# Sthiber/COSC_4397_Pathtracing_Raytracing_Project

Measured on AMD Instinct MI355X. Metric: Msamples/s, cornell.txt 1920x1080 depth 8 (+PSNR vs 5000spp ref), higher is better.
Workload: dtype f32

## Files before the change

### cosc_4397_pathtracing_raytracing_project_amd/csrc/pt_kernels.hip

```cpp
#include "pt_kernels.h"

#include <float.h>

#include <type_traits>

#include "pt_lds.h"
#include "pt_sched.h"
#include "pt_portable_math.h"

#ifndef PT_ARITH
#define PT_ARITH 0
#endif
#if PT_ARITH == 0
#define PT_NS arith_exact
#define PT_API_FN api_exact
#elif PT_ARITH == 1
#define PT_NS arith_fma
#define PT_API_FN api_fma
#elif PT_ARITH == 2
#define PT_NS arith_fast
#define PT_API_FN api_fast
#else
#error "PT_ARITH must be 0, 1 or 2"
#endif
// ... 8 lines not shown
constexpr bool kFloatTrig = PT_ARITH == 1;

#ifdef PT_WALK_STATS
__device__ unsigned long long g_walk_stats[16];
#define PT_STAT(i, v)                                                             \
  do {                                                                            \
    const unsigned long long pt_stat_v = (unsigned long long)(v);  \
    if (lane_id() == 0) atomicAdd(&g_walk_stats[i], pt_stat_v);                   \
  } while (0)
PT_DEV int wave_max_stat(int v) {
  for (int o = 32; o; o >>= 1) v = max(v, __shfl_xor(v, o));
  return v;
}
#else
#define PT_STAT(i, v)
#endif

constexpr int kStealMin = 16;
constexpr int kPrimaryWaves = 5;

typedef float v4f __attribute__((ext_vector_type(4)));
struct f3 {
  float x, y, z;
};
PT_DEV unsigned long long ballot(bool p) { return __builtin_amdgcn_ballot_w64(p); }
PT_DEV uint32_t push_bit(uint32_t m, bool bit) {
  uint32_t r;
  unsigned long long carry_out;
  asm("v_addc_co_u32_e64 %0, %1, %2, %2, %3" : "=v"(r), "=s"(carry_out) : "v"(m), "s"(ballot(bit)));
  return r;
}
PT_DEV int rank_in(unsigned long long m) { return __builtin_amdgcn_mbcnt_hi((uint32_t)(m >> 32), __builtin_amdgcn_mbcnt_lo((uint32_t)m, 0)); }
PT_DEV f3 mk(float x, float y, float z) { return f3{x, y, z}; }

#include "pt_ieee.inc"
PT_DEV void divmod(int a, int n, float inv_n, int& q, int& r) {
  int k = (int)((float)a * inv_n);
  int rem = a - k * n;
  if (rem < 0) {
    rem += n;
    --k;
  } else if (rem >= n) {
    rem -= n;
    ++k;
  }
  q = k;
  r = rem;
}

struct RayInv {
  float ix, iy, iz;
  bool sx, sy, sz;
  float nx, ny, nz;
};

}

#pragma clang fp contract(off)
namespace ex {
namespace {
constexpr bool kFastArith = false, kFusedRef = false;
#include "pt_arith.inc"
}
}
#if PT_ARITH != 0
#pragma clang fp contract(fast)
#endif
namespace md {
namespace {
constexpr bool kFastArith = kFast, kFusedRef = PT_ARITH == 1;
#include "pt_arith.inc"
}
}
namespace {
using namespace md;
constexpr bool kD0 = PT_ARITH != 0;
template <bool EX>
struct Ar {
  static PT_DEV RayInv ray_inv(f3 d, f3 o) { if constexpr (EX) return ex::ray_inv(d, o); else return md::ray_inv(d, o); }
  static PT_DEV bool slab(f3 o, const RayInv& ri, float a, float b, float c, float d, float e, float f) {
    if constexpr (EX) return ex::slab(o, ri, a, b, c, d, e, f); else return md::slab(o, ri, a, b, c, d, e, f);
  }
  static PT_DEV bool slab_rel(const RayInv& ri, float a, float b, float c, float d, float e, float f) {
    if constexpr (EX) return ex::slab_rel(ri, a, b, c, d, e, f); else return md::slab_rel(ri, a, b, c, d, e, f);
  }
  static PT_DEV bool slab_t(f3 o, const RayInv& ri, float a, float b, float c, float d, float e, float f, float& tn) {
    if constexpr (EX) return ex::slab_t(o, ri, a, b, c, d, e, f, tn); else return md::slab_t(o, ri, a, b, c, d, e, f, tn);
  }
  template <int TYPE, bool QO, bool DEFER = false>
  static PT_DEV float geom_test(const ptd::Geom* __restrict__ G, f3 ro, f3 rd, f3& point, f3& normal, f3 qo_pre, int rt_type = -1) {
    if constexpr (EX) return ex::geom_test<TYPE, QO, DEFER>(G, ro, rd, point, normal, qo_pre, rt_type);
    else return md::geom_test<TYPE, QO, DEFER>(G, ro, rd, point, normal, qo_pre, rt_type);
  }
  static PT_DEV f3 finish_normal(const ptd::Geom* __restrict__ G, f3 stored) {
    if constexpr (EX) return ex::finish_normal(G, stored); else return md::finish_normal(G, stored);
  }
  static PT_DEV f3 camera_dir(const ptd::Camera& cam, float inv_w, int p, bool aa, float jx, float jy) {
    if constexpr (EX) return ex::camera_dir(cam, inv_w, p, aa, jx, jy); else return md::camera_dir(cam, inv_w, p, aa, jx, jy);
  }
  static PT_DEV f3 xf_point(const float* m, f3 v) { if constexpr (EX) return ex::mulMV<1>(m, v); else return md::mulMV<1>(m, v); }
};

PT_DEV int lane_id() { return (int)(threadIdx.x & 63); }
PT_DEV float bperm(int src_lane, float v) {
  return __int_as_float(__builtin_amdgcn_ds_bpermute(src_lane << 2, __float_as_int(v)));
}

PT_DEV uint32_t utilhash(uint32_t a) {
  a = (a + 0x7ed55d16u) + (a << 12);
  a = (a ^ 0xc761c23cu) ^ (a >> 19);
  a = (a + 0x165667b1u) + (a << 5);
  a = (a + 0xd3a2646cu) ^ (a << 9);
  a = (a + 0xfd7046c5u) + (a << 3);
  a = (a ^ 0xb55a4f09u) ^ (a >> 16);
  return a;
}
struct MinStd {
  uint32_t x;
  PT_DEV explicit MinStd(uint32_t s) {
    uint32_t r = (s & 0x7fffffffu) + (s >> 31);
    if (r >= 0x7fffffffu) r -= 0x7fffffffu;
    x = r == 0u ? 1u : r;
  }
  PT_DEV uint32_t next() {
    uint64_t p = (uint64_t)x * 48271u;
    uint32_t r = (uint32_t)(p & 0x7fffffffu) + (uint32_t)(p >> 31);
    if (r >= 0x7fffffffu) r -= 0x7fffffffu;
    x = r;
    return r;
  }
  PT_DEV float u01() { return (float)(next() - 1u) * 4.656612873077392578125e-10f; }
};
PT_DEV uint32_t iter_hash(int iter, int depth) { return utilhash((1u << 31) | ((uint32_t)depth << 22) | (uint32_t)iter); }
PT_DEV void iter_hash_fill(uint32_t* tab, const SceneTables& sc, const BatchInfo& b, int depth) {
  if (iter_hash_entries(sc) > 0)
    for (int i = threadIdx.x; i < b.K; i += blockDim.x) tab[i] = iter_hash(b.iter_first + i, depth);
}
PT_DEV uint32_t iter_hash_of(const uint32_t* tab, const SceneTables& sc, const BatchInfo& b, int depth, int k) {
  return iter_hash_entries(sc) > 0 ? tab[k] : iter_hash(b.iter_first + k, depth);
}

PT_DEV void aa_jitter(int iter, int pixel, float& jx, float& jy) {
  MinStd rng(utilhash((1u << 31) | (1u << 30) | (uint32_t)iter) ^ utilhash((uint32_t)pixel));
  jx = rng.u01() - 0.5f;
  jy = rng.u01() - 0.5f;
}

PT_DEV void stage16(void* lds, const void* g, int bytes) {
  const float4* src = reinterpret_cast<const float4*>(g);
  float4* dst = reinterpret_cast<float4*>(lds);
  for (int i = threadIdx.x; i < bytes / 16; i += blockDim.x) dst[i] = src[i];
}

PT_DEV int global_pixel(const BatchInfo& b, int p) {
  if (b.stripe == 0) return b.pixel_begin + p;
  if (b.list) return b.pixel_begin + b.list[p];
  int i, r;
  divmod(p, b.stripe, b.inv_stripe, i, r);
  return b.pixel_begin + p + i * b.gap;
}

struct PathTag {
  int slot;
  uint32_t phash;
  int k;
};
struct PathRec {
  f3 o, d, c;
  PathTag tag;
};
struct alignas(8) Word2 {
  float x, y;
};
PT_DEV void plane2_load(const ptd::PathBuf& b, int64_t at, float& cz, PathTag& tag) {
  const Word2 w2 = reinterpret_cast<const Word2*>(b.r + 2 * b.stride)[at];
  cz = w2.x;
  tag.slot = __float_as_int(w2.y), tag.phash = 0u, tag.k = 0;
}
PT_DEV void plane2_store(const ptd::PathBuf& b, int64_t at, float cz, const PathTag& tag) {
  reinterpret_cast<Word2*>(b.r + 2 * b.stride)[at] = Word2{cz, __int_as_float(tag.slot)};
}
PT_DEV void path_load_ray(const ptd::PathBuf& b, int64_t at, f3& o, f3& d) {
  const ptd::Word4 w0 = b.r[at], w1 = b.r[b.stride + at];
  o = mk(w0.x, w0.y, w0.z);
  d = mk(w0.w, w1.x, w1.y);
}
PT_DEV void path_load_tail(const ptd::PathBuf& b, int64_t at, f3& d, f3& c, PathTag& tag) {
  const ptd::Word4 w1 = b.r[b.stride + at];
  float cz;
  plane2_load(b, at, cz, tag);
  d = mk(reinterpret_cast<const float*>(b.r + at)[3], w1.x, w1.y);
  c = mk(w1.z, w1.w, cz);
}
PT_DEV PathRec path_load(const ptd::PathBuf& b, int64_t at) {
  const ptd::Word4 w0 = b.r[at], w1 = b.r[b.stride + at];
  PathRec v;
  float cz;
  plane2_load(b, at, cz, v.tag);
  v.o = mk(w0.x, w0.y, w0.z);
  v.d = mk(w0.w, w1.x, w1.y);
  v.c = mk(w1.z, w1.w, cz);
  return v;
}
PT_DEV void path_store(const ptd::PathBuf& b, int64_t at, f3 o, f3 d, f3 c, const PathTag& tag) {
  b.r[at] = ptd::Word4{o.x, o.y, o.z, d.x};
  b.r[b.stride + at] = ptd::Word4{d.y, d.z, c.x, c.y};
  plane2_store(b, at, c.z, tag);
}
PT_DEV int make_slot(const BatchInfo& b, int k, int pl) { return (k << b.slot_shift) | pl; }
PT_DEV void sample_of(const PathTag& tag, const BatchInfo& b, int& k, int& pl) {
  k = (int)((uint32_t)tag.slot >> b.slot_shift);
  pl = tag.slot & ((1 << b.slot_shift) - 1);
}
PT_DEV uint32_t path_seed(int k, int pl, const uint32_t* ihash, const SceneTables& sc, const BatchInfo& b, int depth) {
  return iter_hash_of(ihash, sc, b, depth, k) ^ utilhash((uint32_t)global_pixel(b, pl));
}

struct Retire {
  ptd::Word4* rec;
  unsigned long long* sub;
  unsigned long long* cnt;
  int seg_cap, wq0;
};
PT_DEV Retire retire_of(const ptd::RetireBuf& rb, int q) {
  Retire rt;
  rt.rec = rb.rec + (int64_t)q * rb.kmax * rb.seg_cap;
  rt.sub = rb.sub + (int64_t)q * rb.kmax * rb.wq0;
  rt.cnt = rb.cnt + (int64_t)q * rb.kmax;
  rt.seg_cap = rb.seg_cap, rt.wq0 = rb.wq0;
  return rt;
}
PT_DEV void retire_store(const Retire& rt, bool dead, int k, int pos, int pl, f3 c) {
  if (dead) rt.rec[(int64_t)k * rt.seg_cap + pos] = ptd::Word4{c.x, c.y, c.z, __int_as_float(pl)};
}
PT_DEV void retire_append(const Retire& rt, bool dead, int k, int pl, f3 c) {
  if (dead) retire_store(rt, true, k, (int)(atomicAdd(&rt.cnt[k], 1ull << 32) >> 32), pl, c);
}

__global__ __launch_bounds__(kBlock) void k_generate(ptd::Camera cam, BatchInfo b, ptd::Queues qs, ptd::PathBuf out,
                                                     int32_t* __restrict__ cnt0) {
  const int wave = blockIdx.x * kWavesPerBlock + (threadIdx.x >> 6);
  const int lane = lane_id();
  const auto [q, r, wq] = wave_slot(wave, qs.Q, qs.W);
  const float inv_w = 1.0f / (float)cam.res_x;
  const QueueShare sh = queue_share(b, qs, q);
  if (r == 0 && lane == 0) cnt0[cnt_index(qs, 0, q)] = b.K * sh.my_pixels;
  const int entries = b.K * sh.my_nq;
  for (int j = r; j < entries; j += wq) {
    int k, jj;
    divmod(j, sh.my_nq, sh.inv_my_nq, k, jj);
    const int pl = chunk_pixel(q, jj, qs.Q) + lane;
    if (pl < b.N) {
      const int p = global_pixel(b, pl);
      float jx = 0.f, jy = 0.f;
      if (b.aa_jitter) aa_jitter(b.iter_first + k, p, jx, jy);
      const f3 d = Ar<kD0>::camera_dir(cam, inv_w, p, b.aa_jitter != 0, jx, jy);
      const int64_t at = (int64_t)q * qs.cap + (int64_t)k * sh.my_pixels + jj * 64 + lane;
      path_store(out, at, mk(cam.pos[0], cam.pos[1], cam.pos[2]), d, mk(1.0f, 1.0f, 1.0f), PathTag{make_slot(b, k, pl), utilhash((uint32_t)p), k});
    }
  }
}

struct HitRec {
  float t;
  f3 n;
  f3 p;
  int geom;
};

PT_DEV uint32_t permute_xor(uint32_t x, uint32_t m) {
  if (m & 1u) x = ((x & 0x55555555u) << 1) | ((x >> 1) & 0x55555555u);
  if (m & 2u) x = ((x & 0x33333333u) << 2) | ((x >> 2) & 0x33333333u);
  if (m & 4u) x = ((x & 0x0f0f0f0fu) << 4) | ((x >> 4) & 0x0f0f0f0fu);
  if (m & 8u) x = ((x & 0x00ff00ffu) << 8) | ((x >> 8) & 0x00ff00ffu);
  if (m & 16u) x = (x << 16) | (x >> 16);
  return x;
}
PT_DEV uint32_t octant_mask(const RayInv& ri, unsigned long long top_xor) {
  const int oct = (int)ri.sx | ((int)ri.sy << 1) | ((int)ri.sz << 2);
  return (uint32_t)(top_xor >> (oct * 8)) & 31u;
}

template <bool EX = false, typename NP = const v4f*>
PT_DEV void scan_step(NP nodes4, f3 o, const RayInv& ri, bool act, int& cur, float bt,
                      bool& cand, int& leaf, int& geom) {
  const int at_n = act ? cur : 0;
  const v4f NA = nodes4[2 * at_n];
  const v4f NB = nodes4[2 * at_n + 1];
  float tn;
  const bool in = act && Ar<EX>::slab_t(o, ri, NA.x, NA.y, NA.z, NA.w, NB.x, NB.y, tn) && !(tn > bt);
  geom = __float_as_int(NB.w);
  cand = in && geom >= 0;
  leaf = at_n;
  if (act) cur = in ? cur + 1 : __float_as_int(NB.z);
}

struct Walker {
  int cur, end;
  int own;
  f3 o;
  RayInv ri;
};
PT_DEV void steal_step(Walker& w, uint32_t& pend, uint32_t xm, bool idle, unsigned long long I, int* slot,
                       const float4* top, int lane) {
  const unsigned long long Dn = ballot(pend != 0);
  if (!Dn) return;
  const int nd = __popcll(Dn), ni = __popcll(I);
  const int drank = rank_in(Dn);
  const int irank = rank_in(I);
  if (pend != 0) slot[drank] = lane;
  const bool take = idle && irank < nd;
  const int donor = slot[take ? irank : 0];
  const uint32_t dpend = (uint32_t)__builtin_amdgcn_ds_bpermute(donor << 2, (int)pend);
// ... 832 lines not shown
    if (plan.pieces == 1) break;
    int nx = 0;
    if (lane == 0) nx = atomicAdd(&qs.deal[deal_map(qs).strand_counter()], 1);
    strand = qs.W + __builtin_amdgcn_readfirstlane(nx);
  }
}

constexpr int kPathsWaves = 6;
constexpr int kPathsMinReady = 32;
PT_DEV uint32_t lds_offset(const void* p) { return (uint32_t)(uintptr_t)(__attribute__((address_space(3))) const char*)p; }
template <typename T>
PT_DEV const T* uniform_ptr(const T* p) {
  const uint64_t v = (uint64_t)(uintptr_t)p;
  const uint32_t lo = (uint32_t)__builtin_amdgcn_readfirstlane((int)(uint32_t)v), hi = (uint32_t)__builtin_amdgcn_readfirstlane((int)(uint32_t)(v >> 32));
  return reinterpret_cast<const T*>((uintptr_t)(((uint64_t)hi << 32) | lo));
}
PT_DEV void fetch_record_to_lds(const void* b0, const void* b1, const void* b2, int i, uint32_t lds_base) {
  uint32_t keep;
  const uint32_t off16 = (uint32_t)i << 4, off8 = (uint32_t)i << 3;
  asm volatile(
      "s_mov_b32 %[keep], m0\n\t"
      "s_mov_b32 m0, %[base]\n\t"
      "s_nop 0\n\t"
      "global_load_lds_dwordx4 %[o16], %[b0]\n\t"
      "s_add_u32 m0, m0, 0x400\n\t"
      "s_nop 0\n\t"
      "global_load_lds_dwordx4 %[o16], %[b1]\n\t"
      "s_add_u32 m0, m0, 0x400\n\t"
      "s_nop 0\n\t"
      "global_load_lds_dword %[o8], %[b2]\n\t"
      "s_add_u32 m0, m0, 0xfc\n\t"
      "s_nop 0\n\t"
      "global_load_lds_dword %[o8], %[b2] offset:4\n\t"
      "s_mov_b32 m0, %[keep]"
      : [keep] "=&s"(keep)
      : [base] "s"(lds_base), [b0] "s"(b0), [b1] "s"(b1), [b2] "s"(b2), [o16] "v"(off16), [o8] "v"(off8)
      : "memory", "scc");
}
PT_DEV void fetch_split_to_lds(const void* b0, const void* b1, int i, int i0, uint32_t lds_base) {
  uint32_t keep;
  const uint32_t off = (uint32_t)i << 4, off0 = (uint32_t)i0 << 4;
  asm volatile(
      "s_mov_b32 %[keep], m0\n\t"
      "s_mov_b32 m0, %[base]\n\t"
      "s_nop 0\n\t"
      "global_load_lds_dwordx4 %[o], %[b0]\n\t"
      "s_add_u32 m0, m0, 0x400\n\t"
      "s_nop 0\n\t"
      "global_load_lds_dwordx4 %[o0], %[b1]\n\t"
      "s_mov_b32 m0, %[keep]"
      : [keep] "=&s"(keep)
      : [base] "s"(lds_base), [b0] "s"(b0), [b1] "s"(b1), [o] "v"(off), [o0] "v"(off0)
      : "memory", "scc");
}
PT_DEV void read_record_slot(uint32_t s16, uint32_t s4, v4f& w0, v4f& w1, float& cz, int& nslot, int& nrs) {
  asm volatile(
      "s_waitcnt vmcnt(0)\n\t"
      "ds_read_b128 %0, %5\n\t"
      "ds_read_b128 %1, %5 offset:1024\n\t"
      "ds_read_b32 %2, %6\n\t"
      "ds_read_b32 %3, %6 offset:256\n\t"
      "ds_read_b32 %4, %6 offset:512\n\t"
      "s_waitcnt lgkmcnt(0)"
      : "=&v"(w0), "=&v"(w1), "=&v"(cz), "=&v"(nslot), "=&v"(nrs)
      : "v"(s16), "v"(s4)
      : "memory");
}
struct Lanes {
  unsigned long long* best;
  float* rec;
  uint16_t* ent;
  int head, count;
  int appended, processed;
};
PT_DEV Lanes lanes_init(char* base) {
  Lanes c;
  c.best = reinterpret_cast<unsigned long long*>(base + LanesMap::best);
  c.rec = reinterpret_cast<float*>(base + LanesMap::rec);
  c.ent = reinterpret_cast<uint16_t*>(base + LanesMap::ent);
  c.head = c.count = c.appended = c.processed = 0;
  return c;
}
PT_DEV void paths_chunk(Lanes& c, int n, int lane, f3 o, f3 d, const uint32_t* tword, const ptd::Geom* __restrict__ geoms) {
  const bool valid = lane < n;
  const uint32_t entry = c.ent[(c.head + lane) & (kRing - 1)];
  const int src = (int)(entry & 63u);
  const uint32_t tw = tword[valid ? entry >> 6 : 0u];
  const uint32_t leaf = tw & 255u;
  const f3 ro = mk(bperm(src, o.x), bperm(src, o.y), bperm(src, o.z));
  const f3 rd = mk(bperm(src, d.x), bperm(src, d.y), bperm(src, d.z));
  const ptd::Geom* G = geoms + (valid ? (int)(tw >> 8) : 0);
  f3 pt = mk(0.f, 0.f, 0.f), nrm = mk(0.f, 0.f, 0.f);
  const float t = geom_test<-1, false>(G, ro, rd, pt, nrm, mk(0.f, 0.f, 0.f));
  const uint32_t tb = __float_as_uint(t);
  if (valid && t > 0.f && tb < 0x7f7fffffu) {
    const unsigned long long key = ((unsigned long long)tb << 32) | leaf;
    unsigned long long* slot = &c.best[src];
    atomicMin(slot, key);
    if (*slot == key) {
      float* r = c.rec + src;
      r[0 * 64] = nrm.x, r[1 * 64] = nrm.y, r[2 * 64] = nrm.z;
      r[3 * 64] = pt.x, r[4 * 64] = pt.y, r[5 * 64] = pt.z;
    }
  }
  c.head = (c.head + n) & (kRing - 1);
  c.count -= n;
  c.processed += n;
}
typedef __attribute__((address_space(4))) const v4f cfloat4;
template <typename TOP>
PT_DEV void paths_search(Lanes& c, TOP* top, const uint32_t* tword, int ntop, const ptd::Geom* __restrict__ geoms, f3 o, f3 d,
                         bool fresh, int lane, int& mark) {
  const RayInv ri = ray_inv(d, o);
  if (fresh) {
    c.best[lane] = kNoHit;
    mark = c.processed;
  }
  uint32_t mask = 0;
  for (int e0 = 0; e0 < ntop; e0 += 8) {
#pragma unroll
    for (int u = 0; u < 8; ++u) {
      const int e = e0 + u;
      if (e < ntop) {
        const auto A = top[2 * e], B = top[2 * e + 1];
        mask = push_bit(mask, slab(o, ri, A.x, A.y, A.z, A.w, B.x, B.y));
      }
    }
  }
  mask = fresh ? mask : 0u;
  while (true) {
    const unsigned long long m = ballot(mask != 0u);
    if (!m) break;
    const int rank = rank_in(m);
    if (mask != 0u) {
      const int te = ntop - 1 - __builtin_ctz(mask);
      mask &= mask - 1u;
      c.ent[(c.head + c.count + rank) & (kRing - 1)] = (uint16_t)((te << 6) | lane);
      if (mask == 0u) mark = c.appended + rank + 1;
    }
    const int cnt = __popcll(m);
    c.count += cnt;
    c.appended += cnt;
    if (c.count >= 64) paths_chunk(c, 64, lane, o, d, tword, geoms);
  }
}
constexpr int kPathsScanWaves = 5, kPathsGridWaves = 5;
constexpr int kVisitLap = 32, kVisitsPerRefill = 31;
static_assert(kVisitLap + kVisitsPerRefill + 1 <= kVisitRing, "the visit ring laps a path in flight");
static_assert((kVisitRing & (kVisitRing - 1)) == 0, "visit numbers wrap with a mask");
constexpr int kInlineGroup = 8;
template <int GROUP>
PT_DEV void stream_gather_slot(int N, int K, const QueueShare& sh, const ptd::RetireBuf& ret, const ptd::Word4* plane, const ptd::Word4* front,
                               float* __restrict__ image, int q, int s);
template <typename T, typename... R>
PT_DEV const T& first_of(const T& t, const R&...) { return t; }
template <Search MODE, int SPLIT = 0, typename... PREV>
__global__ __launch_bounds__(kBlock, MODE == 0 ? kPathsWaves : MODE == 1 ? kPathsScanWaves : kPathsGridWaves) void k_paths(SceneTables sc, BatchInfo b, ptd::Queues qs, int32_t* __restrict__ cnt ,
                                                               ptd::PathBuf in, ptd::RetireBuf ret, PREV... prev) {
  extern __shared__ float4 lds_raw[];
  char* lds = reinterpret_cast<char*>(lds_raw);
  const PathsLds L = paths_lds<MODE, kFast>(sc);
  stage16(lds + L.top, sc.top_b, MODE == 2 ? 0 : top_bytes(sc));
  stage16(lds + L.mats, sc.mats, mat_bytes(sc));
  const float4* top = reinterpret_cast<const float4*>(lds + L.top);
  const ptd::Mat* mats = reinterpret_cast<const ptd::Mat*>(lds + L.mats);
  const ptd::Node* nodes = sc.nodes_b;
  const ptd::Geom* geoms = sc.geoms;
  if (MODE == 0) {
    stage16(lds + L.geoms, sc.geoms, geom_bytes(sc));
    geoms = reinterpret_cast<const ptd::Geom*>(lds + L.geoms);
  }
  const char* lnodes = nullptr;
  if (MODE == 1 && sc.scan_nodes_lds > 0) {
    stage16(lds + L.nodes, sc.nodes_b, node_bytes(sc));
    lnodes = lds + L.nodes;
  }
  using WM = PathsWaveMap<MODE, kFast>;
  constexpr bool FIXED = SPLIT == kFixedSlots, FIRST = SPLIT == kFirstBounce || FIXED;
  constexpr bool GATHER = sizeof...(PREV) > 0;
  static_assert(!GATHER || FIXED, "only a batch with fixed record slots gathers its predecessor");
  const int he = iter_hash_entries(sc);
  uint32_t* tword = reinterpret_cast<uint32_t*>(lds + L.tword);
  int* lmat = reinterpret_cast<int*>(lds + L.lmat);
  uint32_t* ihash = reinterpret_cast<uint32_t*>(lds + L.ihash);
  for (int d = 1; d < b.trace_depth; ++d) iter_hash_fill(ihash + (d - 1) * he, sc, b, d);
  for (int e = threadIdx.x; MODE == 0 && e < sc.num_top; e += blockDim.x) {
    const int leaf = sc.top[e].idx, gi = sc.nodes[leaf].geom;
    tword[e] = (uint32_t)leaf | ((uint32_t)gi << 8);
    lmat[leaf & 63] = sc.geoms[gi].material;
  }
  __syncthreads();
  const int wib = threadIdx.x >> 6;
  char* wbase = lds + L.waves + wib * L.wave_bytes;
  Lanes cy = lanes_init(wbase);
  GridRings gr = grid_rings_init<false>(wbase);
  Carry<false, 1>& cb = gr.cy;
  CellRing& cr = gr.cr;
  cb.lnodes = (const __attribute__((address_space(3))) v4f*)(lnodes ? lnodes : lds), cb.lds_nodes = lnodes != nullptr;
  constexpr bool SLOTS = MODE == 0;
  char* slots = wbase + WM::slots;
  int* died = reinterpret_cast<int*>(wbase + WM::died);
  [[maybe_unused]] int* fillc = reinterpret_cast<int*>(wbase + WM::fillc);
  const int ntop = sc.num_top;
  const int wave = __builtin_amdgcn_readfirstlane(blockIdx.x * kWavesPerBlock + wib);
  const int lane = lane_id();
  died[lane] = 0;
  const uint64_t t_begin = __builtin_amdgcn_s_memrealtime();
  const DealMap dm = deal_map(qs);
  const WaveSlot even = wave_slot(wave, qs.Q, qs.W);
  int q = even.q, r = even.r, wq = even.wq;
  if (qs.deal != nullptr && qs.deal[dm.made_for()] == qs.W) {
    int at_or_before = 0;
    for (int e0 = 0; e0 < qs.Q; e0 += 64) at_or_before += (int)__popcll(ballot(e0 + lane < qs.Q && qs.deal[dm.first(e0 + lane)] <= wave));
    q = at_or_before - 1;
    const int first = qs.deal[dm.first(q)];
    r = wave - first, wq = qs.deal[dm.first(q + 1)] - first;
  }
  const Retire rt = retire_of(ret, q);
  const int64_t qbase = (int64_t)q * qs.cap;
  const int wq0 = rt.wq0, ne = b.K * wq0;
  const QueueShare qshare = queue_share(b, qs, q);
  const int my_nq = qshare.my_nq, quo = my_nq / wq0, rem = my_nq % wq0;
  auto count_of = [&](int e) { return e < ne ? (int)(uint32_t)rt.sub[e] : 0; };
  int total = 0, csum = 0;
  const bool chunk_sums = ne <= 64 * 64;
  for (int e0 = 0; e0 < ne; e0 += 256) {
    int n4[4];
#pragma unroll
    for (int j = 0; j < 4; ++j) n4[j] = count_of(e0 + 64 * j + lane);
#pragma unroll
    for (int j = 0; j < 4; ++j) {
      int sum;
      (void)wave_prefix6(n4[j], sum);
      total += sum;
      if (lane == (e0 >> 6) + j) csum = sum;
    }
  }
  if (r == 0 && lane == 0) cnt[cnt_index(qs, 1, q)] = total;
  if constexpr (SPLIT == kFirstBounce || SPLIT == kFixedSlots)
    if (r == 0 && lane == 0) cnt[cnt_index(qs, 0, q)] = b.K * qshare.my_pixels;
  const PiecePlan pieces = piece_plan(total, wq, b.paths_pieces, qs.deal != nullptr, chunk_sums);
  [[maybe_unused]] int clist0 = 0;
  int ce = ne, cstart = total, ccnt = 0, clist = 0;
  int cord = 0;
  [[maybe_unused]] int cur_k = 0;
  [[maybe_unused]] uint32_t cur_h = 0u, next_h = 0u;
  [[maybe_unused]] int crec0 = 0;
  [[maybe_unused]] const int fbits = fixed_bits(rt.seg_cap);
  int win0 = -64;
  unsigned long long wsub = 0ull;
  auto window_to = [&](int e) {
    if (e < win0 || e >= win0 + 64) {
      win0 = e;
      wsub = (e + lane < ne) ? rt.sub[e + lane] : 0ull;
    }
  };
  auto sub_word = [&](int e) -> unsigned long long {
    const uint32_t lo32 = (uint32_t)__builtin_amdgcn_readlane((int)(uint32_t)wsub, e - win0);
    const uint32_t hi32 = (uint32_t)__builtin_amdgcn_readlane((int)(uint32_t)(wsub >> 32), e - win0);
    return ((unsigned long long)hi32 << 32) | lo32;
  };
  window_to(0);
  auto cursor_bases = [&](int first_rank) {
    const int ec = min(ce, ne - 1), ck = ec / wq0, crho = ec - ck * wq0;
    clist = ck * rt.seg_cap + sub_offset(quo, rem, crho) * 64;
    if constexpr (SPLIT != 0) clist0 = invariant_slot(clist, ck, rt.seg_cap);
    if constexpr (FIRST) cur_k = ck, cur_h = iter_hash(b.iter_first + ck, 0);
    window_to(ec);
    const int crec = clist + (int)(uint32_t)(sub_word(ec) >> 32);
    if constexpr (FIXED) crec0 = invariant_slot(crec, ck, rt.seg_cap);
    else if (lane == 0) fillc[cord & (kVisitRing - 1)] = crec + (first_rank - cstart);
  };
  auto seek = [&](int at_rank) {
    int cum = 0, e_begin = 0;
    if (chunk_sums) {
      int all;
      const int cbefore = wave_prefix6(csum, all);
      const unsigned long long here = ballot(csum > 0 && cbefore <= at_rank && at_rank < cbefore + csum);
      if (here) {
        const int l = __builtin_ctzll(here);
        e_begin = l * 64, cum = __builtin_amdgcn_readlane(cbefore, l);
      }
    }
    for (int e0 = e_begin; e0 < ne; e0 += 64) {
      const int n = count_of(e0 + lane);
      int sum;
      const int before = wave_prefix6(n, sum);
      const unsigned long long here = ballot(n > 0 && cum + before <= at_rank && at_rank < cum + before + n);
      if (here) {
        const int l = __builtin_ctzll(here);
        ce = e0 + l, cstart = cum + __builtin_amdgcn_readlane(before, l), ccnt = __builtin_amdgcn_readlane(n, l);
        break;
      }
      cum += sum;
    }
    ++cord;
    cursor_bases(at_rank);
  };
  auto assign = [&](bool want, int rank, int& at, [[maybe_unused]] int& at0, int& rs) -> bool {
    bool pending = want;
    const int cord0 = cord;
    while (true) {
      const bool in = pending && rank < cstart + ccnt;
      if (in) at = clist + (rank - cstart), rs = cord;
      if constexpr (SPLIT != 0)
        if (in) at0 = clist0 + (rank - cstart);
      if constexpr (FIRST)
        if (in) rs = (int)(FIXED ? pack_fixed(cur_k, crec0 + (rank - cstart), fbits) : pack_visit(cur_k, cord)), next_h = cur_h;
      pending = pending && !in;
      if (!ballot(pending) || ce >= ne || (!FIXED && cord - cord0 >= kVisitsPerRefill)) break;
      cstart += ccnt;
      ccnt = 0;
      int nxt = ce + 1;
      while (nxt < ne) {
        window_to(nxt);
        const unsigned long long holds = ballot((uint32_t)wsub != 0u) & (~0ull << (nxt - win0));
        if (holds) {
          nxt = win0 + (int)__builtin_ctzll(holds);
          ccnt = (int)(uint32_t)sub_word(nxt);
          break;
        }
        nxt = win0 + 64;
      }
      ce = min(nxt, ne);
      ++cord;
      cursor_bases(cstart);
    }
    return want && !pending;
  };
  const uint32_t s_base = (uint32_t)__builtin_amdgcn_readfirstlane((int)lds_offset(slots));
  const uint32_t s16 = s_base + (uint32_t)lane * 16u, s4 = s_base + (uint32_t)kSlotTail + (uint32_t)lane * 4u;
  const ptd::Word4 *in0 = uniform_ptr(in.r + qbase), *in1 = uniform_ptr(in.r + in.stride + qbase);
  const float* in2 = uniform_ptr(reinterpret_cast<const float*>(in.r + 2 * in.stride) + 2 * qbase);
  PathRec nx;
  nx.o = nx.d = nx.c = mk(0.f, 0.f, 0.f), nx.tag = PathTag{0, 0u, 0};
  int nx_rs = 0;
  int* slot_rs = reinterpret_cast<int*>(slots + kSlotVisit) + lane;
  auto fetch = [&](int at, [[maybe_unused]] int at0, int rs) {
    if constexpr (SLOTS && SPLIT == kSplitRecords) fetch_split_to_lds(in0, in1, at, at0, s_base), *slot_rs = rs;
    else if constexpr (SLOTS) fetch_record_to_lds(in0, in1, in2, FIRST ? at0 : at, s_base), *slot_rs = rs;
    else if constexpr (SPLIT == kSplitRecords) {
      const ptd::Word4 w0 = in.r[qbase + at], w1 = in.r[in.stride + qbase + at0];
      nx.o = mk(w0.x, w0.y, w0.z), nx.d = mk(w0.w, w1.x, w1.y), nx.c = mk(w1.z, w1.w, 0.f), nx_rs = rs;
    } else nx = path_load(in, qbase + at), nx_rs = rs;
  };
  f3 o = mk(0.f, 0.f, 0.f), d = o, c = o;
  int slot = 0, depth = 1, mark = 0, rslot = 0;
  uint32_t phash = 0u;
  bool valid = false, fresh = false, owes = false;
  bool has_next = false;
  int streamed = 0, p_hi = 0;
  [[maybe_unused]] int gj = r;
  [[maybe_unused]] uint32_t gather_time = 0u;
  [[maybe_unused]] auto gather_step = [&]() {
    if constexpr (GATHER) {
      const PrevGather& pg = first_of(prev...);
      const uint64_t t0 = __builtin_amdgcn_s_memrealtime();
      stream_gather_slot<kInlineGroup>(b.N, pg.K, qshare, ret, pg.rec, pg.plane0, pg.image, q, gj * 64 + lane);
      gj += wq;
      gather_time += (uint32_t)(__builtin_amdgcn_s_memrealtime() - t0);
    }
  };
  while (!FIRST) {
    if (streamed >= p_hi && p_hi >= 0) {
      int nextp = -1;
      if (cord == 0) nextp = r;
      else if (pieces.needs_counter()) {
        int v = 0;
        if (lane == 0) v = atomicAdd(&qs.deal[dm.piece_counter(q)], 1);
        nextp = wq + __builtin_amdgcn_readfirstlane(v);
      }
      const PieceRange pr = pieces.piece_range(nextp);
      if (pr.some) {
        streamed = pr.start, p_hi = pr.end;
        seek(streamed);
      } else {
        p_hi = -1;
      }
    }
    const bool take = !valid && has_next;
    if (ballot(take || owes || (!valid && !has_next && streamed < p_hi))) {
      v4f w0, w1;
      float cz;
      int nslot, nrs;
      if constexpr (SLOTS && SPLIT == kSplitRecords) {
        asm volatile(
            "s_waitcnt vmcnt(0)\n\t"
            "ds_read_b128 %0, %3\n\t"
            "ds_read_b128 %1, %3 offset:1024\n\t"
            "ds_read_b32 %2, %4 offset:512\n\t"
            "s_waitcnt lgkmcnt(0)"
            : "=&v"(w0), "=&v"(w1), "=&v"(nrs)
            : "v"(s16), "v"(s4)
            : "memory");
        cz = 0.f, nslot = 0;
      } else if constexpr (SLOTS) {
        read_record_slot(s16, s4, w0, w1, cz, nslot, nrs);
      } else {
        w0 = v4f{nx.o.x, nx.o.y, nx.o.z, nx.d.x}, w1 = v4f{nx.d.y, nx.d.z, nx.c.x, nx.c.y}, cz = nx.c.z, nslot = nx.tag.slot, nrs = nx_rs;
      }
      if (owes) {
        rt.rec[rslot] = ptd::Word4{c.x, c.y, c.z, __int_as_float(slot & ((1 << b.slot_shift) - 1))};
        owes = false;
      }
      if constexpr (SPLIT == kSplitRecords) {
        if (take) {
          const uint32_t word = __float_as_uint(w0.w);
          const ptd::Mat* m = mats + __float_as_int(w1.w);
          nslot = kind_sample_id(word);
          o = mk(w1.x, w1.y, w1.z), d = mk(w0.x, w0.y, w0.z);
          c = mul(mk(1.0f, 1.0f, 1.0f), kind_specular(word) ? mk(m->spec[0], m->spec[1], m->spec[2]) : mk(m->color[0], m->color[1], m->color[2]));
        }
      } else if (take) o = mk(w0.x, w0.y, w0.z), d = mk(w0.w, w1.x, w1.y), c = mk(w1.z, w1.w, cz);
      if (take) {
        slot = nslot, rslot = nrs;
        phash = utilhash((uint32_t)global_pixel(b, nslot & ((1 << b.slot_shift) - 1)));
        depth = 1;
        valid = fresh = true;
        has_next = false;
      }
      const bool lapping = ballot(valid && cord - rslot >= kVisitLap) != 0ull;
      const bool empty = !has_next && !lapping;
      const unsigned long long em = ballot(empty);
      const int rank = rank_in(em);
      const bool more = empty && streamed + rank < p_hi;
      int at = 0, at0 = 0, rs = 0;
      const bool served = assign(more, streamed + rank, at, at0, rs);
      if (served) {
        has_next = true;
        fetch(at, at0, rs);
      }
      streamed += (int)__popcll(ballot(served));
    }
    if (!ballot(valid || has_next) && p_hi < 0) break;
    bool ready;
    if constexpr (MODE == 0) {
      if (ballot(fresh)) {
        if constexpr (kFast) paths_search(cy, (cfloat4*)(uintptr_t)sc.top_b, tword, ntop, geoms, o, d, fresh, lane, mark);
        else paths_search(cy, top, tword, ntop, geoms, o, d, fresh, lane, mark);
      }
      ready = valid && (cy.processed - mark) >= 0;
      if (cy.count > 0 && __popcll(ballot(ready)) < kPathsMinReady) {
        paths_chunk(cy, cy.count, lane, o, d, tword, geoms);
        ready = valid;
      }
    } else {
      cb.best[lane] = kNoHit;
      if constexpr (MODE == 2) grid_search<1>(cb, cr, sc, nodes, geoms, o, d, valid, lane, 0);
      else {
        PT_STAT(14, 1);
        PT_STAT(15, __popcll(ballot(valid)));
        carry_search<true, 1>(cb, top, ntop, nodes, geoms, o, d, valid, lane, 0, sc.cull_margin, sc.top_xor);
      }
      while (cb.count > 0) carry_chunk<false, 1, false, MODE == 2>(cb, min(64, cb.count), lane, nodes, geoms);
      ready = valid;
    }
    fresh = false;
    {
      ShadeIO s;
      s.o = mk(0.f, 0.f, 0.f);
      s.d = d;
      s.c = c;
      s.alive = false;
      Bounce bo;
      bo.kind = 0;
      const int k = (int)((uint32_t)slot >> b.slot_shift);
      const unsigned long long best = cy.best[lane];
      Hit h{false, -1.0f, -1, 0, mk(0.f, 0.f, 0.f), mk(0.f, 0.f, 0.f)};
      if (ready) {
        if ((uint32_t)(best >> 32) != 0x7f7fffffu) {
          h.t = __uint_as_float((uint32_t)(best >> 32));
          const float* rr = cy.rec + lane;
          h.n = mk(rr[0 * 64], rr[1 * 64], rr[2 * 64]);
          h.p = mk(rr[3 * 64], rr[4 * 64], rr[5 * 64]);
          if constexpr (MODE == 0) {
            h.mat = lmat[(uint32_t)best & 63u];
          } else {
            const ptd::Geom* G = geoms + nodes[(uint32_t)best].geom;
            h.mat = G->material;
            if (MODE == 2) h.n = finish_normal(G, h.n);
          }
        }
        const uint32_t ih = he > 0 ? ihash[(depth - 1) * he + k] : iter_hash(b.iter_first + k, depth);
        bo = shade_decide(mats, b.trace_depth, depth, ih ^ phash, h.t, h.mat, s);
      }
      const bool alive = ready && s.alive, dead = ready && !s.alive;
      if (dead) atomicAdd(&died[depth & 63], 1);
      if (dead) rslot = atomicAdd(&fillc[rslot & (kVisitRing - 1)], 1);
      if (alive) shade_bounce(bo, h.n, h.p, s);
      if (ready) {
        c = s.c;
        if (alive) o = s.o, d = s.d, depth += 1, fresh = true;
        else valid = false, owes = true;
      }
    }
  }
  if constexpr (FIRST) {
    static_assert(MODE == kLdsTables, "the first-bounce form takes its records from the refill slots of the LDS-table form");
    while (true) {
      if (ballot(fresh)) {
        if constexpr (kFast) paths_search(cy, (cfloat4*)(uintptr_t)sc.top_b, tword, ntop, geoms, o, d, fresh, lane, mark);
        else paths_search(cy, top, tword, ntop, geoms, o, d, fresh, lane, mark);
      }
      bool ready = valid && (cy.processed - mark) >= 0;
      if (cy.count > 0 && __popcll(ballot(ready)) < kPathsMinReady) {
        paths_chunk(cy, cy.count, lane, o, d, tword, geoms);
        ready = valid;
      }
      fresh = false;
      Bounce bo;
      bo.kind = 0, bo.rng_x = 1u, bo.roughness = 0.f;
      f3 axis = mk(0.f, 0.f, 0.f);
      bool go = false;
      {
        ShadeIO s;
        s.o = mk(0.f, 0.f, 0.f);
        s.d = d;
        s.c = c;
        s.alive = false;
        const int k = (int)((uint32_t)slot >> b.slot_shift);
        const unsigned long long best = cy.best[lane];
        Hit h{false, -1.0f, -1, 0, mk(0.f, 0.f, 0.f), mk(0.f, 0.f, 0.f)};
        if (ready) {
          if ((uint32_t)(best >> 32) != 0x7f7fffffu) {
            h.t = __uint_as_float((uint32_t)(best >> 32));
            const float* rr = cy.rec + lane;
            h.n = mk(rr[0 * 64], rr[1 * 64], rr[2 * 64]);
            h.p = mk(rr[3 * 64], rr[4 * 64], rr[5 * 64]);
            h.mat = lmat[(uint32_t)best & 63u];
          }
          const uint32_t ih = he > 0 ? ihash[(depth - 1) * he + k] : iter_hash(b.iter_first + k, depth);
          bo = shade_decide(mats, b.trace_depth, depth, ih ^ phash, h.t, h.mat, s);
        }
        const bool alive = ready && s.alive, dead = ready && !s.alive;
        if (dead) atomicAdd(&died[depth & 63], 1);
        if constexpr (!FIXED)
          if (dead) rslot = atomicAdd(&fillc[rslot & (kVisitRing - 1)], 1);
        if (ready) {
          c = s.c;
          if (alive) {
            const BounceAxis a = bounce_axis(bo, h.n, h.p, d);
            o = a.o, axis = a.f, go = true;
          } else valid = false, owes = true;
        }
      }
      if (streamed >= p_hi && p_hi >= 0) {
        if constexpr (GATHER)
          if (cord != 0 && gj < my_nq) gather_step();
        int nextp = -1;
        if (cord == 0) nextp = r;
        else if (pieces.needs_counter()) {
          int v = 0;
          if (lane == 0) v = atomicAdd(&qs.deal[dm.piece_counter(q)], 1);
          nextp = wq + __builtin_amdgcn_readfirstlane(v);
        }
        const PieceRange pr = pieces.piece_range(nextp);
        if (pr.some) {
          streamed = pr.start, p_hi = pr.end;
          seek(streamed);
        } else {
          p_hi = -1;
        }
      }
      const bool take = !valid && has_next;
      if (ballot(take || owes || (!valid && !has_next && streamed < p_hi))) {
        v4f w0, w1;
        float cz;
        int word, vword;
        read_record_slot(s16, s4, w0, w1, cz, word, vword);
        if (owes) {
          rt.rec[rslot] = ptd::Word4{c.x, c.y, c.z, __int_as_float(slot & ((1 << b.slot_shift) - 1))};
          owes = false;
        }
        if (take) {
          const int pl = first_pixel(word, b.slot_shift), k = FIXED ? fixed_k((uint32_t)vword, fbits) : visit_k((uint32_t)vword);
          const f3 hn = mk(w0.w, w1.x, w1.y), cam_d = mk(w1.z, w1.w, cz);
          slot = make_slot(b, k, pl), rslot = FIXED ? fixed_slot_of((uint32_t)vword, fbits, rt.seg_cap) : visit_number((uint32_t)vword);
          phash = utilhash((uint32_t)global_pixel(b, pl));
          ShadeIO s;
          s.o = mk(0.f, 0.f, 0.f);
          s.d = cam_d;
          s.c = mk(1.0f, 1.0f, 1.0f);
          s.alive = false;
          bo = shade_decide(mats, b.trace_depth, 0, next_h ^ phash, 0.0f, first_material(word, b.slot_shift), s);
          o = mk(w0.x, w0.y, w0.z), c = s.c;
          axis = bo.kind == 1 ? bounce_reflect(cam_d, hn) : hn;
          depth = 0;
          valid = go = true;
          has_next = false;
        }
        bool lapping = false;
        if constexpr (!FIXED) lapping = ballot(valid && visit_gap(cord, rslot) >= kVisitLap) != 0ull;
        const bool empty = !has_next && !lapping;
        const unsigned long long em = ballot(empty);
        const int rank = rank_in(em);
        const bool more = empty && streamed + rank < p_hi;
        int at = 0, at0 = 0, rs = 0;
        const bool served = assign(more, streamed + rank, at, at0, rs);
        if (served) {
          has_next = true;
          fetch(at, at0, rs);
        }
        streamed += (int)__popcll(ballot(served));
      }
      if (!ballot(valid || has_next) && p_hi < 0) break;
      if (go) d = bounce_sample(bo, axis), depth += 1, fresh = true;
    }
  }
  if constexpr (GATHER) {
    while (gj < my_nq) gather_step();
    if (r == 0)
      for (int i = lane; i < ret.kmax; i += 64) ret.cnt[(int64_t)q * ret.kmax + i] = 0ull;
  }
  if (lane == 0) {
    int reached = 0, rays = 0;
    for (int dd = min(b.trace_depth - 1, 63); dd >= 2; --dd) {
      reached += died[dd];
      rays += reached;
      if (reached) atomicAdd(&cnt[cnt_index(qs, dd, q)], reached);
    }
    rays += reached + died[1];
    uint64_t spent = __builtin_amdgcn_s_memrealtime() - t_begin;
    if constexpr (GATHER) spent -= min(spent, (uint64_t)gather_time);
    const int ticks = (int)min(spent >> 6, (uint64_t)0x3ffff);
    if (qs.deal != nullptr && rays) atomicAdd(&qs.deal[dm.time(q)], ticks), atomicAdd(&qs.deal[dm.rays(q)], rays);
  }
}

__global__ __launch_bounds__(kBlock) void k_shade_stage(SceneTables sc, int trace_depth, int depth, int n,
                                                        const int32_t* __restrict__ iter,
                                                        const int32_t* __restrict__ pixel, ptd::HitBuf hits,
                                                        ptd::PathBuf paths, int32_t* __restrict__ alive) {
  extern __shared__ float4 lds_raw[];
  char* lds = reinterpret_cast<char*>(lds_raw);
  const ShadeLds L = shade_lds<false>(sc);
  stage16(lds + L.mats, sc.mats, mat_bytes(sc));
  __syncthreads();
  const ptd::Mat* mats = reinterpret_cast<const ptd::Mat*>(lds + L.mats);
  const int64_t HS = hits.stride;
  for (int at = blockIdx.x * blockDim.x + threadIdx.x; at < n; at += gridDim.x * blockDim.x) {
    const PathRec pr = path_load(paths, at);
    ShadeIO s;
    s.o = pr.o;
    s.d = pr.d;
    s.c = pr.c;
    s.alive = false;
    const Bounce bo = shade_decide(mats, trace_depth, depth, iter_hash(iter[at], depth) ^ utilhash((uint32_t)pixel[at]), hits.t[at], hits.mat[at], s);
    if (bo.kind) shade_bounce(bo, mk(hits.n[at], hits.n[HS + at], hits.n[2 * HS + at]),
                              mk(hits.p[at], hits.p[HS + at], hits.p[2 * HS + at]), s);
    path_store(paths, at, s.o, s.d, s.c, pr.tag);
    alive[at] = s.alive ? 1 : 0;
  }
}

#include "pt_features.inc"
#include "pt_output.inc"
#include "pt_launch.inc"
const KernelApi kApi = {
#if PT_ARITH == 0
    "exact",
#elif PT_ARITH == 1
    "fma",
#else
    "fast",
#endif
    launch_generate, launch_primary, launch_intersect, launch_shade, launch_collect, launch_count_stats,
    launch_preview, launch_save_u8, launch_shade_stage, lds_table_limit, resident_blocks_per_cu, launch_ieee_check, launch_paths,
    launch_collect_conv, launch_features, kFast ? 1 : 0, launch_intersect_grid, launch_collect_stream, launch_paths_gather,
    launch_collect_stream_planes};

}
}

const KernelApi* PT_API_FN() { return &PT_NS::kApi; }

#if defined(PT_WALK_STATS) && PT_ARITH == 2
}
extern "C" int pt_debug_walk_stats(unsigned long long* out) {
  unsigned long long zero[16] = {0};
  if (hipDeviceSynchronize() != hipSuccess) return -1;
  if (hipMemcpyFromSymbol(out, HIP_SYMBOL(ptk::arith_fast::g_walk_stats), sizeof(zero)) != hipSuccess) return -1;
  if (hipMemcpyToSymbol(HIP_SYMBOL(ptk::arith_fast::g_walk_stats), zero, sizeof(zero)) != hipSuccess) return -1;
  return 16;
}
namespace ptk {
#endif

}
```

Measured before the change: 42990.

## Reload cold kernel arguments from kernarg segment to cut live scalar registers

In the LDS-table paths kernel, rarely used batch, queue, count and gather arguments are reread through the kernarg segment pointer when needed, behind opaque asm barriers, instead of staying live across the main loop. Piece plans and pixel-map fields are recomputed on the rare refill and piece-switch paths. Contiguous pixel batches get a simple base-plus-offset pixel fast path. The aim is to lower SGPR/VGPR pressure and spills in the hot loop, at the cost of extra scalar loads on the cold paths and code that relies on a hand-mirrored kernarg struct layout.

```diff
diff --git a/cosc_4397_pathtracing_raytracing_project_amd/csrc/pt_kernels.hip b/cosc_4397_pathtracing_raytracing_project_amd/csrc/pt_kernels.hip
--- a/cosc_4397_pathtracing_raytracing_project_amd/csrc/pt_kernels.hip
+++ b/cosc_4397_pathtracing_raytracing_project_amd/csrc/pt_kernels.hip
@@ -184,13 +184,20 @@
   for (int i = threadIdx.x; i < bytes / 16; i += blockDim.x) dst[i] = src[i];
 }
 
-PT_DEV int global_pixel(const BatchInfo& b, int p) {
+struct PixelMap {
+  int pixel_begin, stripe, gap;
+  float inv_stripe;
+  const int32_t* list;
+};
+PT_DEV PixelMap pixel_map(const BatchInfo& b) { return PixelMap{b.pixel_begin, b.stripe, b.gap, b.inv_stripe, b.list}; }
+PT_DEV int global_pixel(const PixelMap& b, int p) {
   if (b.stripe == 0) return b.pixel_begin + p;
   if (b.list) return b.pixel_begin + b.list[p];
   int i, r;
   divmod(p, b.stripe, b.inv_stripe, i, r);
   return b.pixel_begin + p + i * b.gap;
 }
+PT_DEV int global_pixel(const BatchInfo& b, int p) { return global_pixel(pixel_map(b), p); }
 
 struct PathTag {
   int slot;
@@ -1329,8 +1336,32 @@
 template <int GROUP>
 PT_DEV void stream_gather_slot(int N, int K, const QueueShare& sh, const ptd::RetireBuf& ret, const ptd::Word4* plane, const ptd::Word4* front,
                                float* __restrict__ image, int q, int s);
-template <typename T, typename... R>
-PT_DEV const T& first_of(const T& t, const R&...) { return t; }
+template <typename... PREV>
+struct PathsPrev {};
+template <typename P>
+struct PathsPrev<P> {
+  P p;
+};
+template <typename... PREV>
+struct PathsArgs {
+  SceneTables sc;
+  BatchInfo b;
+  ptd::Queues qs;
+  int32_t* cnt;
+  ptd::PathBuf in;
+  ptd::RetireBuf ret;
+  PathsPrev<PREV...> prev;
+};
+template <typename A>
+PT_DEV const A& cold_args() {
+  auto p = __builtin_amdgcn_kernarg_segment_ptr();
+  asm volatile("" : "+s"(p));
+  return *(const A*)p;
+}
+PT_DEV int cold(int v) {
+  asm volatile("" : "+s"(v));
+  return v;
+}
 template <Search MODE, int SPLIT = 0, typename... PREV>
 __global__ __launch_bounds__(kBlock, MODE == 0 ? kPathsWaves : MODE == 1 ? kPathsScanWaves : kPathsGridWaves) void k_paths(SceneTables sc, BatchInfo b, ptd::Queues qs, int32_t* __restrict__ cnt ,
                                                                ptd::PathBuf in, ptd::RetireBuf ret, PREV... prev) {
@@ -1356,6 +1387,16 @@
   constexpr bool FIXED = SPLIT == kFixedSlots, FIRST = SPLIT == kFirstBounce || FIXED;
   constexpr bool GATHER = sizeof...(PREV) > 0;
   static_assert(!GATHER || FIXED, "only a batch with fixed record slots gathers its predecessor");
+  constexpr bool COLD = MODE == kLdsTables;
+  using Args = PathsArgs<PREV...>;
+  auto c_b = [&]() -> const BatchInfo& {
+    if constexpr (COLD) return cold_args<Args>().b;
+    else return b;
+  };
+  auto c_qs = [&]() -> const ptd::Queues& {
+    if constexpr (COLD) return cold_args<Args>().qs;
+    else return qs;
+  };
   const int he = iter_hash_entries(sc);
   uint32_t* tword = reinterpret_cast<uint32_t*>(lds + L.tword);
   int* lmat = reinterpret_cast<int*>(lds + L.lmat);
@@ -1416,7 +1457,11 @@
   if (r == 0 && lane == 0) cnt[cnt_index(qs, 1, q)] = total;
   if constexpr (SPLIT == kFirstBounce || SPLIT == kFixedSlots)
     if (r == 0 && lane == 0) cnt[cnt_index(qs, 0, q)] = b.K * qshare.my_pixels;
-  const PiecePlan pieces = piece_plan(total, wq, b.paths_pieces, qs.deal != nullptr, chunk_sums);
+  const PiecePlan pieces0 = piece_plan(total, wq, b.paths_pieces, qs.deal != nullptr, chunk_sums);
+  auto piece_plan_here = [&]() {
+    if constexpr (COLD) return piece_plan(cold(total), wq, c_b().paths_pieces, c_qs().deal != nullptr, cold(ne) <= 64 * 64);
+    else return pieces0;
+  };
   [[maybe_unused]] int clist0 = 0;
   int ce = ne, cstart = total, ccnt = 0, clist = 0;
   int cord = 0;
@@ -1450,7 +1495,7 @@
   };
   auto seek = [&](int at_rank) {
     int cum = 0, e_begin = 0;
-    if (chunk_sums) {
+    if (COLD ? cold(ne) <= 64 * 64 : chunk_sums) {
       int all;
       const int cbefore = wave_prefix6(csum, all);
       const unsigned long long here = ballot(csum > 0 && cbefore <= at_rank && at_rank < cbefore + csum);
@@ -1521,6 +1566,21 @@
       nx.o = mk(w0.x, w0.y, w0.z), nx.d = mk(w0.w, w1.x, w1.y), nx.c = mk(w1.z, w1.w, 0.f), nx_rs = rs;
     } else nx = path_load(in, qbase + at), nx_rs = rs;
   };
+  const int pix0 = b.stripe == 0 && b.pixel_begin >= 0 ? b.pixel_begin : -1;
+  auto refill_pixel_map = [&]() {
+    PixelMap pm{0, 0, 0, 0.f, nullptr};
+    if constexpr (COLD)
+      if (pix0 < 0) pm = pixel_map(c_b());
+    return pm;
+  };
+  auto pixel_of = [&](const PixelMap& pm, int pl) {
+    if constexpr (COLD) {
+      if (pix0 >= 0) return pix0 + pl;
+      return global_pixel(pm, pl);
+    } else return global_pixel(b, pl);
+  };
+  [[maybe_unused]] uintptr_t top_b_scalar = (uintptr_t)sc.top_b;
+  if constexpr (COLD && kFast) asm volatile("" : "+s"(top_b_scalar));
   f3 o = mk(0.f, 0.f, 0.f), d = o, c = o;
   int slot = 0, depth = 1, mark = 0, rslot = 0;
   uint32_t phash = 0u;
@@ -1531,20 +1591,23 @@
   [[maybe_unused]] uint32_t gather_time = 0u;
   [[maybe_unused]] auto gather_step = [&]() {
     if constexpr (GATHER) {
-      const PrevGather& pg = first_of(prev...);
+      const Args& ka = cold_args<Args>();
+      const PrevGather& pg = ka.prev.p;
+      const int gq = cold(q);
       const uint64_t t0 = __builtin_amdgcn_s_memrealtime();
-      stream_gather_slot<kInlineGroup>(b.N, pg.K, qshare, ret, pg.rec, pg.plane0, pg.image, q, gj * 64 + lane);
+      stream_gather_slot<kInlineGroup>(ka.b.N, pg.K, queue_share(ka.b, ka.qs, gq), ka.ret, pg.rec, pg.plane0, pg.image, gq, gj * 64 + lane);
       gj += wq;
       gather_time += (uint32_t)(__builtin_amdgcn_s_memrealtime() - t0);
     }
   };
   while (!FIRST) {
     if (streamed >= p_hi && p_hi >= 0) {
+      const PiecePlan pieces = piece_plan_here();
       int nextp = -1;
       if (cord == 0) nextp = r;
       else if (pieces.needs_counter()) {
         int v = 0;
-        if (lane == 0) v = atomicAdd(&qs.deal[dm.piece_counter(q)], 1);
+        if (lane == 0) v = atomicAdd(&c_qs().deal[deal_map(c_qs()).piece_counter(q)], 1);
         nextp = wq + __builtin_amdgcn_readfirstlane(v);
       }
       const PieceRange pr = pieces.piece_range(nextp);
@@ -1557,6 +1620,7 @@
     }
     const bool take = !valid && has_next;
     if (ballot(take || owes || (!valid && !has_next && streamed < p_hi))) {
+      const PixelMap pm = refill_pixel_map();
       v4f w0, w1;
       float cz;
       int nslot, nrs;
@@ -1591,7 +1655,7 @@
       } else if (take) o = mk(w0.x, w0.y, w0.z), d = mk(w0.w, w1.x, w1.y), c = mk(w1.z, w1.w, cz);
       if (take) {
         slot = nslot, rslot = nrs;
-        phash = utilhash((uint32_t)global_pixel(b, nslot & ((1 << b.slot_shift) - 1)));
+        phash = utilhash((uint32_t)pixel_of(pm, nslot & ((1 << b.slot_shift) - 1)));
         depth = 1;
         valid = fresh = true;
         has_next = false;
@@ -1613,7 +1677,7 @@
     bool ready;
     if constexpr (MODE == 0) {
       if (ballot(fresh)) {
-        if constexpr (kFast) paths_search(cy, (cfloat4*)(uintptr_t)sc.top_b, tword, ntop, geoms, o, d, fresh, lane, mark);
+        if constexpr (kFast) paths_search(cy, (cfloat4*)top_b_scalar, tword, ntop, geoms, o, d, fresh, lane, mark);
         else paths_search(cy, top, tword, ntop, geoms, o, d, fresh, lane, mark);
       }
       ready = valid && (cy.processed - mark) >= 0;
@@ -1676,7 +1740,7 @@
     static_assert(MODE == kLdsTables, "the first-bounce form takes its records from the refill slots of the LDS-table form");
     while (true) {
       if (ballot(fresh)) {
-        if constexpr (kFast) paths_search(cy, (cfloat4*)(uintptr_t)sc.top_b, tword, ntop, geoms, o, d, fresh, lane, mark);
+        if constexpr (kFast) paths_search(cy, (cfloat4*)top_b_scalar, tword, ntop, geoms, o, d, fresh, lane, mark);
         else paths_search(cy, top, tword, ntop, geoms, o, d, fresh, lane, mark);
       }
       bool ready = valid && (cy.processed - mark) >= 0;
@@ -1721,14 +1785,15 @@
           } else valid = false, owes = true;
         }
       }
-      if (streamed >= p_hi && p_hi >= 0) {
+      if (__builtin_expect(streamed >= p_hi && p_hi >= 0, 0)) {
         if constexpr (GATHER)
           if (cord != 0 && gj < my_nq) gather_step();
+        const PiecePlan pieces = piece_plan_here();
         int nextp = -1;
         if (cord == 0) nextp = r;
         else if (pieces.needs_counter()) {
           int v = 0;
-          if (lane == 0) v = atomicAdd(&qs.deal[dm.piece_counter(q)], 1);
+          if (lane == 0) v = atomicAdd(&c_qs().deal[deal_map(c_qs()).piece_counter(q)], 1);
           nextp = wq + __builtin_amdgcn_readfirstlane(v);
         }
         const PieceRange pr = pieces.piece_range(nextp);
@@ -1741,6 +1806,7 @@
       }
       const bool take = !valid && has_next;
       if (ballot(take || owes || (!valid && !has_next && streamed < p_hi))) {
+        const PixelMap pm = refill_pixel_map();
         v4f w0, w1;
         float cz;
         int word, vword;
@@ -1753,7 +1819,7 @@
           const int pl = first_pixel(word, b.slot_shift), k = FIXED ? fixed_k((uint32_t)vword, fbits) : visit_k((uint32_t)vword);
           const f3 hn = mk(w0.w, w1.x, w1.y), cam_d = mk(w1.z, w1.w, cz);
           slot = make_slot(b, k, pl), rslot = FIXED ? fixed_slot_of((uint32_t)vword, fbits, rt.seg_cap) : visit_number((uint32_t)vword);
-          phash = utilhash((uint32_t)global_pixel(b, pl));
+          phash = utilhash((uint32_t)pixel_of(pm, pl));
           ShadeIO s;
           s.o = mk(0.f, 0.f, 0.f);
           s.d = cam_d;
@@ -1787,22 +1853,31 @@
   if constexpr (GATHER) {
     while (gj < my_nq) gather_step();
     if (r == 0)
-      for (int i = lane; i < ret.kmax; i += 64) ret.cnt[(int64_t)q * ret.kmax + i] = 0ull;
+      for (int i = lane, kmax = cold_args<Args>().ret.kmax; i < kmax; i += 64) cold_args<Args>().ret.cnt[(int64_t)q * kmax + i] = 0ull;
   }
   if (lane == 0) {
     int reached = 0, rays = 0;
-    for (int dd = min(b.trace_depth - 1, 63); dd >= 2; --dd) {
+    int32_t* const ecnt = COLD ? cold_args<Args>().cnt : cnt;
+    for (int dd = min(c_b().trace_depth - 1, 63); dd >= 2; --dd) {
       reached += died[dd];
       rays += reached;
-      if (reached) atomicAdd(&cnt[cnt_index(qs, dd, q)], reached);
+      if (reached) atomicAdd(&ecnt[cnt_index(c_qs(), dd, q)], reached);
     }
     rays += reached + died[1];
     uint64_t spent = __builtin_amdgcn_s_memrealtime() - t_begin;
     if constexpr (GATHER) spent -= min(spent, (uint64_t)gather_time);
     const int ticks = (int)min(spent >> 6, (uint64_t)0x3ffff);
-    if (qs.deal != nullptr && rays) atomicAdd(&qs.deal[dm.time(q)], ticks), atomicAdd(&qs.deal[dm.rays(q)], rays);
-  }
-}
+    const ptd::Queues& eq = c_qs();
+    if (eq.deal != nullptr && rays) atomicAdd(&eq.deal[deal_map(eq).time(q)], ticks), atomicAdd(&eq.deal[deal_map(eq).rays(q)], rays);
+  }
+}
+
+template <typename... PREV>
+using PathsSignature = void (*)(decltype(PathsArgs<PREV...>::sc), decltype(PathsArgs<PREV...>::b), decltype(PathsArgs<PREV...>::qs), decltype(PathsArgs<PREV...>::cnt),
+                                decltype(PathsArgs<PREV...>::in), decltype(PathsArgs<PREV...>::ret), PREV...);
+static_assert(std::is_same<decltype(&k_paths<kLdsTables, kFixedSlots>), PathsSignature<>>::value, "PathsArgs does not mirror k_paths' arguments");
+static_assert(std::is_same<decltype(&k_paths<kLdsTables, kFixedSlots, PrevGather>), PathsSignature<PrevGather>>::value, "PathsArgs does not mirror k_paths' arguments");
+static_assert(std::is_same<decltype(PathsArgs<PrevGather>::prev.p), PrevGather>::value && std::is_standard_layout<PathsArgs<PrevGather>>::value, "PathsArgs: the gathered batch comes last");
 
 __global__ __launch_bounds__(kBlock) void k_shade_stage(SceneTables sc, int trace_depth, int depth, int n,
                                                         const int32_t* __restrict__ iter,
```

Result: faster. 43790, median of 6 (+1.9%).
